# csm-kr/faster_rcnn_pytorch

Measured on AMD Instinct MI355X. Metric: train images/sec (VGG16 Faster R-CNN, 600x1000, bs=1/GPU), higher is better.
Workload: dtype f32; 1 GPU; VGG16 Faster R-CNN train step, synthetic 600x1000 frames, bs=1/GPU, HIP proposal/RoI path (N=20646 anchors, pre/post NMS 12000/2000, 128 RoIs, RoIPool 7x7 on 512x37x62); global_batch=1, parallelism=dp1, submission=eager (one launch per kernel), sampling=device-philox

## Files before the change

faster_rcnn_pytorch_amd/_lib.py:

```python
import ctypes as C
import os

_HERE = os.path.dirname(os.path.abspath(__file__))
LIB_PATH = os.environ.get("FRCNN_HIP_LIB") or os.path.join(_HERE, "lib", "libfrcnn_hip.so")

OK = 0
ABI_VERSION = 7
HT_ERR_PERM_LENGTH, HT_ERR_PERM_RANGE, HT_ERR_UPSTREAM_ABORT, HT_ERR_SHORT = 1, 2, 4, 8
HT_ERR_GT_COUNT = RPN_ERR_GT_COUNT = 16
OP_TOPK, OP_NMS, OP_REGION_PROPOSAL, OP_RPN_TARGETS, OP_HEAD_TARGETS, OP_PREPROCESS, OP_HEAD_BWD, OP_RPN_CONV, OP_RPN_CONV_WGRAD, OP_RPN_CONV_F32 = 1, 2, 3, 4, 5, 6, 7, 8, 9, 10
OP_DETECT = 11
OP_EVAL = 12
OP_COCO_EVAL = 13
OP_EVAL_MERGE = 14
OP_COCO_EVAL_POOLED = 15
OP_DETECT_MERGE = 16
MERGE_COUNT_CLIPPED, MERGE_UPSTREAM_ABORT, MERGE_LABEL_RANGE, MERGE_CLASS_OVERFLOW, MERGE_OUTPUT_OVERFLOW = 1, 2, 4, 8, 16
MERGE_MAX_SETS, MERGE_MAX_CANDIDATES = 8, 2048
SOFT_NMS_HARD, SOFT_NMS_LINEAR, SOFT_NMS_GAUSSIAN = 0, 1, 2
EVAL_TP, EVAL_FP, EVAL_IGNORED = 1, 2, 3
EVAL_ERR_UPSTREAM_ABORT, EVAL_ERR_GT_OVERFLOW, EVAL_ERR_COUNT_RANGE, EVAL_ERR_LABEL_RANGE = 1, 2, 4, 8
EVAL_ERR_LEDGER_OVERFLOW = 16
EVAL_ERR_SHARD_TRUNCATED = 32
EVAL_MERGE_MAX_SHARDS = 64
SGD_CHUNK = 8192

_vp, _i, _i64, _f, _u64, _sz = C.c_void_p, C.c_int, C.c_int64, C.c_float, C.c_uint64, C.c_size_t

SIGNATURES = {
    "frcnn_abi_version": (_i, []),
    "frcnn_layout_check": (_i, []),
    "frcnn_layout_stamp": (_u64, []),
    "frcnn_last_error": (C.c_char_p, []),
    "frcnn_workspace_bytes": (_sz, [_i, _i64, _i64]),
    "frcnn_anchor_base_host": (_i, [_i, _vp, _i, _vp, _i, _vp]),
    "frcnn_tv_base_anchors_host": (_i, [_f, _vp, _i, _vp]),
    "frcnn_anchor_grid": (_i, [_i, _vp, _vp, _vp, _vp, _vp, _i, _f, _f, _vp, _i64, _vp]),
    "frcnn_box_codec": (_i, [_i, _vp, _vp, _i64, _vp, _vp]),
    "frcnn_pairwise_iou": (_i, [_vp, _i64, _vp, _i64, _f, _vp, _vp]),
    "frcnn_proposal_prologue": (_i, [_vp, _vp, _vp, _i64, _f, _vp, _vp, _vp]),
    "frcnn_topk_sorted": (_i, [_vp, _vp, _i64, _i64, _vp, _vp, _vp, _vp, _vp, _sz, _vp]),
    "frcnn_argsort_desc": (_i, [_vp, _vp, _i64, _vp, _vp, _vp, _vp, _vp, _sz, _vp]),
    "frcnn_nms": (_i, [_vp, _vp, _i64, _f, _i64, _vp, _vp, _vp, _vp, _sz, _vp]),
    "frcnn_nms_classed": (_i, [_vp, _vp, _vp, _i64, _f, _i64, _vp, _vp, _vp, _vp, _sz, _vp]),
    "frcnn_region_proposal": (_i, [_vp, _vp, _vp, _i64, _i, _i, _i, _vp, _i, _f, _f, _f, _i64, _f, _i64, _vp, _i, _vp, _vp, _vp, _vp, _sz, _vp]),
    "frcnn_rpn_head_tail_fwd": (_i, [_vp, _i, _i64, _vp, _vp, _vp, _i, _vp, _vp, _i, _vp, _vp, _vp]),
    "frcnn_rpn_head_tail_ml_fwd": (_i, [_vp, _i, _i, _i, _vp, _i, _vp, _vp, _vp, _i, _vp, _vp, _i, _vp, _vp, _vp]),
    "frcnn_rpn_head_tail_ml_bwd": (_i, [_vp, _vp, _i, _i, _vp, _i, _vp, _vp, _i, _vp, _i, _vp, _vp, _vp, _vp, _vp, _vp, _vp, _vp, _sz, _vp]),
    "frcnn_rpn_conv_head_fwd": (_i, [_vp, _vp, _vp, _vp, _i, _i, _vp, _vp, _vp, _vp, _i, _vp, _vp, _i, _vp, _vp, _vp, _sz, _vp]),
    "frcnn_rpn_conv_bwd_data": (_i, [_vp, _vp, _vp, _vp, _i, _i, _vp, _vp, _sz, _vp]),
    "frcnn_rpn_conv_wgrad": (_i, [_vp, _vp, _vp, _vp, _i, _i, _vp, _vp, _sz, _vp]),
    "frcnn_rpn_conv3x3_f32_workspace": (_sz, [_vp, _vp, _i, _i]),
    "frcnn_gemm_nt_f32_workspace": (_sz, []),
    "frcnn_gemm_nt_f32": (_i, [_vp, _vp, _vp, _i, _i, _i, _i, _vp, _sz, _vp]),
    "frcnn_affine_act_fwd": (_i, [_vp, _vp, _vp, _vp, _vp, _i, _i, _i, _vp]),
    "frcnn_affine_act_bwd": (_i, [_vp, _vp, _vp, _vp, _vp, _i, _i, _i, _vp]),
    "frcnn_affine_act_fwd_mixed": (_i, [_vp, _i, _vp, _vp, _i, _vp, _vp, _vp, _i, _i, _i, _vp]),
    "frcnn_affine_act_bwd_mixed": (_i, [_vp, _i, _vp, _vp, _vp, _vp, _i, _vp, _i, _i, _i, _vp]),
    "frcnn_conv3x3_c3_fwd": (_i, [_vp, _vp, _i, _i, _i, _vp, _vp, _i, _vp, _vp]),
    "frcnn_conv3x3_c3_wgrad_workspace": (_sz, [_i, _i]),
    "frcnn_conv3x3_c3_wgrad": (_i, [_vp, _vp, _i, _i, _i, _vp, _vp, _vp, _vp, _sz, _vp]),
    "frcnn_conv3x3_f32_workspace": (_sz, [_vp, _vp, _i, _i, _i]),
    "frcnn_conv3x3_f32_xt_floats": (_sz, [_vp, _vp, _i, _i]),
    "frcnn_conv3x3_f32_relu_bits_words": (_sz, [_vp, _vp, _i, _i]),
    "frcnn_conv3x3_f32_u_floats": (_sz, [_vp, _vp, _i, _i, _i]),
    "frcnn_conv3x3_f32_products": (_i, [_i]),
    "frcnn_conv3x3_f32_fwd": (_i, [_vp, _vp, _vp, _vp, _i, _i, _i, _vp, _vp, _i, _vp, _vp, _vp, _vp, _sz, _vp]),
    "frcnn_conv3x3_f32_tile_size": (_i, [_vp, _vp, _i]),
    "frcnn_conv3x3_f32_supported": (_i, [_vp, _vp, _i, _i, _i, _i]),
    "frcnn_conv3x3_f32_plan": (_i, [_vp, _vp, _i, _i, _i, _vp, _i]),
    "frcnn_conv3x3_f32_bwd_data": (_i, [_vp, _vp, _vp, _vp, _vp, _i, _i, _i, _vp, _vp, _i, _vp, _i, _vp, _sz, _vp]),
    "frcnn_conv3x3_f32_wgrad": (_i, [_vp, _vp, _vp, _vp, _vp, _i, _i, _i, _vp, _vp, _vp, _i, _vp, _vp, _sz, _vp]),
    "frcnn_conv3x3_f32_bwd": (_i, [_vp, _vp, _vp, _vp, _vp, _i, _i, _i, _vp, _vp, _i, _vp, _vp, _vp, _vp, _vp, _sz, _vp]),
    "frcnn_rpn_conv3x3_f32_fwd": (_i, [_vp, _vp, _vp, _vp, _i, _i, _vp, _vp, _sz, _vp]),
    "frcnn_rpn_conv3x3_f32_bwd_data": (_i, [_vp, _vp, _vp, _vp, _i, _i, _vp, _vp, _sz, _vp]),
    "frcnn_rpn_conv3x3_f32_wgrad": (_i, [_vp, _vp, _vp, _vp, _i, _i, _vp, _vp, _sz, _vp]),
    "frcnn_rpn_targets": (_i, [_i, _vp, _i64, _vp, _i64, _vp, _i64, _vp, _i64, _u64, _u64, _vp, _vp, _vp, _vp, _vp, _sz, _vp]),
    "frcnn_head_targets": (_i, [_i, _vp, _vp, _i64, _vp, _vp, _i64, _i64, _i64, _i64, _vp, _i64, _vp, _i64, _u64, _u64, _vp,
                                _vp, _vp, _vp, _vp, _vp, _vp, _vp]),
    "frcnn_rpn_targets_n": (_i, [_i, _vp, _i64, _vp, _i64, _vp, _vp, _i64, _vp, _i64, _u64, _u64, _vp, _vp, _vp, _vp, _vp, _sz, _vp]),
    "frcnn_head_targets_n": (_i, [_i, _vp, _vp, _i64, _vp, _vp, _i64, _vp, _i64, _i64, _i64, _vp, _i64, _vp, _i64, _u64, _u64, _vp,
                                  _vp, _vp, _vp, _vp, _vp, _vp, _vp, _vp]),
    "frcnn_roi_pool_fwd": (_i, [_vp, _i, _i, _i, _vp, _i64, _i, _i, _f, _vp, _vp, _vp]),
    "frcnn_roi_pool_bwd": (_i, [_vp, _vp, _i64, _i, _i, _i, _i, _i, _vp, _vp]),
    "frcnn_roi_pool_fwd_a16": (_i, [_vp, _i, _i, _i, _vp, _i64, _f, _vp, _vp, _vp]),
    "frcnn_roi_pool_bwd_a16": (_i, [_vp, _vp, _vp, _f, _i64, _i, _i, _i, _vp, _vp]),
    "frcnn_roi_pool_plan": (_i, [_i, _i, _i, _i64, _i, _i, _i, _i, _vp, _i]),
    "frcnn_roi_level_map": (_i, [_vp, _i64, _i, _i, _f, _i, _f, _vp, _vp]),
    "frcnn_ms_roi_align_fwd": (_i, [_vp, _vp, _vp, _vp, _i, _i, _vp, _i64, _i, _i, _i, _i, _i, _f, _i, _vp, _vp, _vp, _vp]),
    "frcnn_roi_scale_order": (_i, [_vp, _i64, _vp, _vp, _vp, _vp, _i, _i, _i, _f, _i, _vp, _vp, _vp, _vp]),
    "frcnn_ms_roi_align_bwd": (_i, [_vp, _vp, _vp, _vp, _vp, _i, _i, _vp, _i64, _i, _i, _i, _i, _i, _f, _i, _vp, _sz, _vp]),
    "frcnn_ms_roi_align_bwd_workspace": (_sz, [_vp, _vp, _i, _i, _i64]),
    "frcnn_detection_loss": (_i, [_vp, _vp, _vp, _vp, _i64, _vp, _vp, _vp, _vp, _i64, _i, _vp, _vp, _vp, _vp, _vp, _vp, _sz, _vp]),
    "frcnn_detect_postprocess": (_i, [_vp, _vp, _vp, _vp, _i64, _i, _f, _vp, _f, _vp, _vp, _vp, _vp, _vp, _vp, _vp, _sz, _vp]),
    "frcnn_detect_merge": (_i, [_i, _vp, _vp, _vp, _vp, _vp, _vp, _i, _f, _f, _f, _vp, _vp, _vp, _vp, _vp, _vp, _i64, _vp, _sz, _vp]),
    "frcnn_detect_merge_soft": (_i, [_i, _vp, _vp, _vp, _vp, _vp, _vp, _i, _f, _f, _f, _i, _f, _f, _vp, _vp, _vp, _vp, _vp, _vp, _i64, _vp, _sz, _vp]),
    "frcnn_eval_update": (_i, [_vp, _vp, _vp, _vp, _i64, _vp, _vp, _vp, _vp, _i64, _vp, _vp, _i, _i, _vp, _vp, _vp, _vp, _vp, _vp, _i64, _vp, _vp,
                                _vp, _sz, _vp]),
    "frcnn_eval_average_precision": (_i, [_vp, _vp, _vp, _i64, _vp, _i, _i, _vp, _vp, _vp, _vp, _sz, _vp]),
    "frcnn_coco_eval_update": (_i, [_vp, _vp, _vp, _vp, _i64, _vp, _vp, _vp, _vp, _vp, _i64, _vp, _vp, _i, _i, _i, _vp, _vp, _vp, _vp, _vp, _vp, _i64,
                                     _vp, _vp, _vp, _sz, _vp]),
    "frcnn_coco_eval_update_pooled": (_i, [_vp, _vp, _vp, _vp, _i64, _vp, _vp, _vp, _vp, _vp, _i64, _vp, _vp, _i, _i, _i, _vp, _vp, _vp, _vp, _vp, _vp,
                                            _i64, _vp, _vp, _vp, _sz, _vp]),
    "frcnn_coco_eval_accumulate": (_i, [_vp, _vp, _vp, _vp, _i64, _vp, _vp, _i, _i, _i, _i, _i, _i, _vp, _vp, _vp, _sz, _vp]),
    "frcnn_eval_ledger_append": (_i, [_vp, _vp, _vp, _i64, _vp, _vp, _vp, _vp, _vp, _i64, _vp, _vp, _vp]),
    "frcnn_eval_merge": (_i, [_i, _i64, _i64, _i, _i64] + [_vp] * 11 + [_vp] * 5 + [_i64] + [_vp] * 3 + [_i64] + [_vp] * 6 + [_vp, _sz, _vp]),
    "frcnn_preprocess_image": (_i, [_vp, _i, _i, _i, _i, _i, _i, _i, _vp, _vp, _vp, _vp, _vp, _sz, _vp]),
    "frcnn_preprocess_boxes": (_i, [_vp, _i64, _i, _i, _i, _i, _i, _vp, _vp]),
    "frcnn_mosaic_workspace": (_sz, [_vp, _i, _i]),
    "frcnn_mosaic": (_i, [_vp, _vp, _i, _i, _vp, _vp, _vp, _vp, _vp, _vp, _vp, _vp, _vp, _vp, _sz, _vp]),
    "frcnn_photometric_workspace": (_sz, [_i, _i]),
# ... 106 lines not shown
```

faster_rcnn_pytorch_amd/csrc/conv_c3.hip:

```cpp
#include "frcnn_common.h"
#include "frcnn_dev.h"
#include "frcnn_internal.h"
#include "frcnn_layout.h"
FRCNN_LAYOUT_STAMP(conv_c3);

#define C3_TW 256

__global__ __launch_bounds__(256) void conv3x3_c3_fwd_kernel(const float *__restrict__ x, float *__restrict__ y, int H, int W, int Cout,
                                                             const float *__restrict__ w, const float *__restrict__ bias, int relu,
                                                             unsigned long long *__restrict__ bits)
{
    __shared__ float s[9][C3_TW + 4];
    extern __shared__ __attribute__((aligned(16))) float sw[];
    const int row = blockIdx.y, x0 = blockIdx.x * C3_TW, tid = threadIdx.x;
    for (int e = tid; e < Cout * 28; e += 256) {
        const int co = e / 28, k = e - co * 28;
        sw[e] = k < 27 ? w[(size_t)co * 27 + k] : (bias ? bias[co] : 0.0f);
    }
    {
        float v[10];
#pragma unroll
        for (int j = 0; j < 10; ++j) {
            const int e = tid + 256 * j, r = e / (C3_TW + 2), q = e - r * (C3_TW + 2), ci = r / 3, ky = r - 3 * ci, yy = row - 1 + ky, xx = x0 - 1 + q;
            v[j] = (r < 9 && yy >= 0 && yy < H && xx >= 0 && xx < W) ? x[((size_t)ci * H + yy) * W + xx] : 0.0f;
        }
#pragma unroll
        for (int j = 0; j < 10; ++j) {
            const int e = tid + 256 * j, r = e / (C3_TW + 2), q = e - r * (C3_TW + 2);
            if (r < 9) s[r][q] = v[j];
        }
    }
    __syncthreads();
    const int xx = x0 + tid;
    if (xx >= W) return;
    float v[27];
#pragma unroll
    for (int r = 0; r < 9; ++r)
#pragma unroll
        for (int kx = 0; kx < 3; ++kx) v[r * 3 + kx] = s[r][tid + kx];
    float *yo = y + (size_t)row * W + xx;
    const size_t plane = (size_t)H * W;
    unsigned long long word = 0;
    for (int c2 = 0; c2 < Cout; c2 += 2) {
        const bool two = c2 + 1 < Cout;
        const float4 *w0 = (const float4 *)&sw[c2 * 28], *w1 = (const float4 *)&sw[(two ? c2 + 1 : c2) * 28];
        float acc0 = sw[c2 * 28 + 27], acc1 = sw[(two ? c2 + 1 : c2) * 28 + 27];
#pragma unroll
        for (int q = 0; q < 7; ++q) {
            const float4 a = w0[q], c = w1[q];
            const float aw[4] = {a.x, a.y, a.z, a.w}, cw[4] = {c.x, c.y, c.z, c.w};
#pragma unroll
            for (int e = 0; e < 4; ++e)
                if (q * 4 + e < 27) { acc0 = fmaf(aw[e], v[q * 4 + e], acc0); acc1 = fmaf(cw[e], v[q * 4 + e], acc1); }
        }
#pragma unroll
        for (int j = 0; j < 2; ++j) {
            const int co = c2 + j;
            if (co < Cout) {
                const float pre = j ? acc1 : acc0, o = relu && pre < 0.0f ? 0.0f : pre;
                yo[(size_t)co * plane] = o;
                word |= o > 0.0f ? 1ull << (co & 63) : 0ull;
                if (bits && ((co & 63) == 63 || co == Cout - 1)) { bits[(size_t)(co >> 6) * plane + (size_t)row * W + xx] = word; word = 0; }
            }
        }
    }
}

#define C3_WAVES 8
#define C3_CPW 4
template <bool BITS>
__global__ __launch_bounds__(64 * C3_WAVES) void conv3x3_c3_wgrad_kernel(const float *__restrict__ x, const float *__restrict__ dy, int H, int W, int Cout,
                                                                       const unsigned long long *__restrict__ bits, float *__restrict__ part, int rows)
{
    extern __shared__ float s[];
    const int tid = threadIdx.x, lane = tid & 63, wave = tid >> 6, ws = W + 2, NT = 64 * C3_WAVES;
    const int co0 = (blockIdx.y * C3_WAVES + wave) * C3_CPW;
    const size_t plane = (size_t)H * W;
    typedef float c3_f32x2 __attribute__((ext_vector_type(2)));
    c3_f32x2 acc[C3_CPW][14];
#pragma unroll
    for (int j = 0; j < C3_CPW; ++j)
#pragma unroll
        for (int k = 0; k < 14; ++k) acc[j][k] = (c3_f32x2){0.0f, 0.0f};
    const int r0 = blockIdx.x * rows, nrow = min(rows, H - r0), RS = rows + 2, n_el = 3 * RS * ws;
    for (int base = tid; base < n_el; base += NT * 8) {
        float v[8];
#pragma unroll
        for (int j = 0; j < 8; ++j) {
            const int e = base + NT * j, rr = e / ws, q = e - rr * ws, ci = rr / RS, ry = rr - RS * ci, yy = r0 - 1 + ry, xx = q - 1;
            v[j] = (e < n_el && yy >= 0 && yy < H && xx >= 0 && xx < W) ? x[((size_t)ci * H + yy) * W + xx] : 0.0f;
        }
#pragma unroll
        for (int j = 0; j < 8; ++j) {
            const int e = base + NT * j;
            if (e < n_el) s[e] = v[j];
        }
    }
    __syncthreads();
    if (co0 >= Cout) return;
    const int nxb = (W + 255) / 256;
    auto load = [&](int ry, int xb, float (&gq)[4][C3_CPW], unsigned (&mq)[4]) {
        const float *g0 = dy + (size_t)co0 * plane + (size_t)(r0 + ry) * W;
        const unsigned *b0 = BITS ? (const unsigned *)(bits + (size_t)(co0 >> 6) * plane + (size_t)(r0 + ry) * W) + ((co0 & 63) >> 5) : nullptr;
#pragma unroll
        for (int i = 0; i < 4; ++i) {
            const int xc = min(xb + 64 * i + lane, W - 1);
            mq[i] = BITS ? b0[2 * xc] : ~0u;
#pragma unroll
            for (int j = 0; j < C3_CPW; ++j) gq[i][j] = g0[(size_t)j * plane + xc];
        }
    };
    float g[4][C3_CPW];
    unsigned mb[4];
    load(0, 0, g, mb);
    for (int ry = 0, xbi = 0;;) {
        const int xb = xbi * 256;
        int ry2 = ry, xbi2 = xbi + 1;
        if (xbi2 == nxb) { xbi2 = 0; ++ry2; }
        const bool more = ry2 < nrow;
        float gn[4][C3_CPW];
        unsigned mn[4];
        if (more) load(ry2, xbi2 * 256, gn, mn);
#pragma unroll
        for (int i = 0; i < 4; ++i) {
            const int xx = xb + 64 * i + lane;
            if (xb + 64 * i < W) {
                float v[27];
                const int xc = xx < W ? xx : W - 1;
#pragma unroll
                for (int r = 0; r < 9; ++r)
#pragma unroll
                    for (int kx = 0; kx < 3; ++kx) v[r * 3 + kx] = s[((r / 3) * RS + ry + r % 3) * ws + xc + kx];
#pragma unroll
                for (int j = 0; j < C3_CPW; ++j) {
                    const float gg = (xx < W && (!BITS || ((mb[i] >> ((co0 & 31) + j)) & 1u))) ? g[i][j] : 0.0f;
#pragma unroll
                    for (int k = 0; k < 14; ++k) {
                        const c3_f32x2 vv = {v[2 * k], k < 13 ? v[2 * k + 1] : 1.0f}, g2 = {gg, gg};
                        acc[j][k] = __builtin_elementwise_fma(g2, vv, acc[j][k]);
                    }
                }
            }
        }
        if (!more) break;
#pragma unroll
        for (int i = 0; i < 4; ++i) {
            mb[i] = mn[i];
#pragma unroll
            for (int j = 0; j < C3_CPW; ++j) g[i][j] = gn[i][j];
        }
        ry = ry2; xbi = xbi2;
    }
#pragma unroll
    for (int j = 0; j < C3_CPW; ++j)
#pragma unroll
        for (int k = 0; k < 28; ++k) {
            const float t = wave_sum_dpp(acc[j][k >> 1][k & 1]);
            if (lane == 63) part[((size_t)blockIdx.x * Cout + co0 + j) * 28 + k] = t;
        }
}

__global__ __launch_bounds__(256) void conv3x3_c3_wgrad_finalize_kernel(const float *__restrict__ part, int H, int Cout, float *__restrict__ dw,
                                                                        float *__restrict__ db)
{
    const int o = blockIdx.x * 256 + threadIdx.x;
    if (o >= Cout * 28) return;
    const size_t stride = (size_t)Cout * 28;
    float t = 0.0f;
    int r = 0;
    for (; r + 8 <= H; r += 8) {
        float v[8];
#pragma unroll
        for (int j = 0; j < 8; ++j) v[j] = part[(size_t)(r + j) * stride + o];
#pragma unroll
        for (int j = 0; j < 8; ++j) t += v[j];
    }
    for (; r < H; ++r) t += part[(size_t)r * stride + o];
    const int co = o / 28, k = o - co * 28;
    if (k < 27) dw[(size_t)co * 27 + k] = t;
    else if (db) db[co] = t;
}

static int c3_check(const void *x, const void *y, int H, int W, int Cout, const void *w, const char *what)
{
    FRCNN_REQUIRE(x && y && w, "%s: NULL pointer", what);
    FRCNN_REQUIRE(H > 0 && W > 0 && Cout > 0 && Cout <= 256 && (long long)H * W * Cout < (1ll << 31), "%s: bad size %d x %d x %d", what, Cout, H, W);
    return FRCNN_OK;
}

FRCNN_EXPORT int frcnn_conv3x3_c3_fwd(const float *x_dev, float *y_dev, int H, int W, int Cout, const float *w_dev, const float *bias_dev, int relu,
                                      unsigned long long *relu_bits_dev, void *stream)
{
    int rc = c3_check(x_dev, y_dev, H, W, Cout, w_dev, "conv3x3_c3_fwd");
    if (rc) return rc;
    FRCNN_LAUNCH(conv3x3_c3_fwd_kernel, dim3((unsigned)((W + C3_TW - 1) / C3_TW), (unsigned)H), dim3(256), (size_t)Cout * 28 * sizeof(float), (hipStream_t)stream, x_dev, y_dev, H, W, Cout,
                 w_dev, bias_dev, relu, relu_bits_dev);
    FRCNN_CHECK_LAUNCH("conv3x3_c3_fwd_kernel");
    return FRCNN_OK;
}

FRCNN_EXPORT size_t frcnn_conv3x3_c3_wgrad_workspace(int H, int Cout)
{
    return (H > 0 && Cout > 0) ? (size_t)H * Cout * 28 * sizeof(float) : 0;
}

FRCNN_EXPORT int frcnn_conv3x3_c3_wgrad(const float *x_dev, const float *dy_dev, int H, int W, int Cout, const unsigned long long *relu_bits_dev,
                                        float *dw_dev, float *dbias_dev, void *workspace, size_t workspace_bytes, void *stream)
{
    int rc = c3_check(x_dev, dy_dev, H, W, Cout, dw_dev, "conv3x3_c3_wgrad");
    if (rc) return rc;
    FRCNN_REQUIRE(dw_dev && workspace, "conv3x3_c3_wgrad: NULL pointer");
    if (Cout % 4 != 0 || W > 1700)
        return frcnn_set_error(FRCNN_ERR_UNSUPPORTED, "conv3x3_c3_wgrad: Cout = %d must be a multiple of 4 and W = %d at most 1700", Cout, W);
    if (workspace_bytes < frcnn_conv3x3_c3_wgrad_workspace(H, Cout))
        return frcnn_set_error(FRCNN_ERR_WORKSPACE, "conv3x3_c3_wgrad: workspace %zu < %zu bytes", workspace_bytes, frcnn_conv3x3_c3_wgrad_workspace(H, Cout));
    hipStream_t s = (hipStream_t)stream;
    float *part = (float *)workspace;
    const int groups = (Cout + C3_CPW * C3_WAVES - 1) / (C3_CPW * C3_WAVES);
    int cus = 256, dev = 0;
    if (hipGetDevice(&dev) == hipSuccess) (void)hipDeviceGetAttribute(&cus, hipDeviceAttributeMultiprocessorCount, dev);
    const int fit = (int)((150 * 1024) / (12 * (size_t)(W + 2))) - 2;
    const int rows = std::max(1, std::min(fit, (int)(((long long)H * groups + cus - 1) / cus)));
    const int nb = (H + rows - 1) / rows;
    const dim3 wg((unsigned)nb, (unsigned)groups);
    const size_t wl = (size_t)3 * (rows + 2) * (W + 2) * sizeof(float);
    if (relu_bits_dev) (void)hipFuncSetAttribute((const void *)conv3x3_c3_wgrad_kernel<true>, hipFuncAttributeMaxDynamicSharedMemorySize, (int)wl);
    else (void)hipFuncSetAttribute((const void *)conv3x3_c3_wgrad_kernel<false>, hipFuncAttributeMaxDynamicSharedMemorySize, (int)wl);
    if (relu_bits_dev) FRCNN_LAUNCH(conv3x3_c3_wgrad_kernel<true>, wg, dim3(64 * C3_WAVES), wl, s, x_dev, dy_dev, H, W, Cout, relu_bits_dev, part, rows);
    else FRCNN_LAUNCH(conv3x3_c3_wgrad_kernel<false>, wg, dim3(64 * C3_WAVES), wl, s, x_dev, dy_dev, H, W, Cout, relu_bits_dev, part, rows);
    FRCNN_CHECK_LAUNCH("conv3x3_c3_wgrad_kernel");
    FRCNN_LAUNCH(conv3x3_c3_wgrad_finalize_kernel, dim3((unsigned)((Cout * 28 + 255) / 256)), dim3(256), 0, s, part, nb, Cout, dw_dev, dbias_dev);
    FRCNN_CHECK_LAUNCH("conv3x3_c3_wgrad_finalize_kernel");
    return FRCNN_OK;
}
```

faster_rcnn_pytorch_amd/ops.py:

```python
import collections
import ctypes as C

import numpy as np
import torch

from . import _lib
from ._lib import check, lib


def _stream():
    return C.c_void_p(torch.cuda.current_stream().cuda_stream)


def _ptr(t):
    return C.c_void_p(0 if t is None else t.data_ptr())


def _req(t, dtype=torch.float32, name="tensor"):
    if not isinstance(t, torch.Tensor):
        raise TypeError("%s must be a torch.Tensor" % name)
    if not t.is_cuda:
        raise RuntimeError("%s is on %s: the frcnn ops run only on a HIP device (no CPU fallback)" % (name, t.device))
    if t.dtype != dtype:
        raise TypeError("%s must be %s, got %s" % (name, dtype, t.dtype))
# ... 1238 lines not shown
        if x.dtype not in (torch.bfloat16, torch.float32) or not x.is_cuda:
            raise ValueError("affine_act_mixed: x must be a bf16 or fp32 HIP tensor")
        x = x.contiguous()
        Cc, HW = int(x.shape[1]), int(x.shape[2] * x.shape[3])
        if res is not None:
            res = _req(res, name="res")
            if res.shape != x.shape:
                raise ValueError("affine_act_mixed: residual and input differ in shape")
        ctx.set_materialize_grads(False)
        y = torch.empty_like(x, dtype=torch.bfloat16 if out_bf16 else torch.float32)
        twin = torch.empty_like(x, dtype=torch.bfloat16) if want_twin else None
        with torch.cuda.device(x.device):
            check(lib.frcnn_affine_act_fwd_mixed(_ptr(x), 1 if x.dtype == torch.bfloat16 else 0, _ptr(res), _ptr(y), 1 if out_bf16 else 0, _ptr(twin),
                                                 _ptr(scale), _ptr(shift), Cc, HW, 1 if relu else 0, _stream()), "affine_act_fwd_mixed")
        _affine_trace("affine_act_fwd_mixed_kernel", x, res, y, twin, scale, shift)
        ctx.relu, ctx.has_res, ctx.x_bf16, ctx.twin = bool(relu), res is not None, x.dtype == torch.bfloat16, bool(want_twin)
        ctx.save_for_backward(scale, y if relu else None)
        if want_twin:
            return y, twin
        return y

    @staticmethod
    def backward(ctx, g, g2=None):
        scale, y = ctx.saved_tensors
        need_x, need_r = ctx.needs_input_grad[5], ctx.has_res and ctx.needs_input_grad[6]
        if not need_x and not need_r:
            return None, None, None, None, None, None, None
        if g is None and g2 is None:
            return None, None, None, None, None, None, None
        if g is None:
            g = torch.zeros_like(g2, dtype=torch.float32)
        g = g.contiguous()
        if g2 is not None:
            g2 = g2.contiguous()
        Cc, HW = int(g.shape[1]), int(g.shape[2] * g.shape[3])
        dx = torch.empty_like(g, dtype=torch.bfloat16 if ctx.x_bf16 else torch.float32)
        dres = torch.empty_like(g, dtype=torch.float32) if (need_r and (ctx.relu or g2 is not None or g.dtype != torch.float32)) else None
        with torch.cuda.device(g.device):
            check(lib.frcnn_affine_act_bwd_mixed(_ptr(g), 1 if g.dtype == torch.bfloat16 else 0, _ptr(g2), _ptr(y), _ptr(scale), _ptr(dx),
                                                 1 if ctx.x_bf16 else 0, _ptr(dres), Cc, HW, 1 if ctx.relu else 0, _stream()), "affine_act_bwd_mixed")
        _affine_trace("affine_act_bwd_mixed_kernel", g, g2, y, dx, dres, scale)
        return None, None, None, None, None, (dx if need_x else None), ((dres if dres is not None else g) if need_r else None)


def affine_act_mixed(x, scale, shift, res=None, relu=False, out_bf16=False, twin=False):
    return _AffineActMixedFn.apply(bool(relu), bool(out_bf16), bool(twin), scale.reshape(-1), shift.reshape(-1), x, res)


def affine_act_mixed_supported(x):
    return (x.is_cuda and x.dtype in (torch.bfloat16, torch.float32) and x.dim() == 4 and x.shape[0] == 1 and torch.is_autocast_enabled()
            and torch.get_autocast_dtype("cuda") == torch.bfloat16)


def conv3x3_c3_fwd(x, w, bias=None, relu=False, want_bits=False):
    x, w = _req(x, name="x"), _req(w, name="w")
    if x.dim() != 4 or x.shape[0] != 1 or x.shape[1] != 3 or w.dim() != 4 or tuple(w.shape[1:]) != (3, 3, 3):
        raise ValueError("conv3x3_c3: x must be [1,3,h,w] and w [Cout,3,3,3]")
    Cout, H, W = int(w.shape[0]), int(x.shape[2]), int(x.shape[3])
    if bias is not None:
        bias = _req(bias, name="bias")
    y = torch.empty((1, Cout, H, W), dtype=torch.float32, device=x.device)
    bits = torch.empty(((Cout + 63) // 64, H, W), dtype=torch.int64, device=x.device) if want_bits else None
    with torch.cuda.device(x.device):
        check(lib.frcnn_conv3x3_c3_fwd(_ptr(x), _ptr(y), H, W, Cout, _ptr(w), _ptr(bias), 1 if relu else 0, _ptr(bits), _stream()), "conv3x3_c3_fwd")
    return (y, bits) if want_bits else y


def conv3x3_c3_wgrad(x, dy, relu_bits=None, want_bias=True):
    x, dy = _req(x, name="x"), _req(dy, name="dy")
    Cout, H, W = int(dy.shape[1]), int(x.shape[2]), int(x.shape[3])
    if x.dim() != 4 or x.shape[0] != 1 or x.shape[1] != 3 or tuple(dy.shape) != (1, Cout, H, W):
        raise ValueError("conv3x3_c3_wgrad: x must be [1,3,h,w] and dy [1,Cout,h,w]")
    if relu_bits is not None:
        relu_bits = _req(relu_bits, torch.int64, "relu_bits")
        if tuple(relu_bits.shape) != ((Cout + 63) // 64, H, W):
            raise ValueError("conv3x3_c3_wgrad: relu_bits does not belong to these shapes")
    dw = torch.empty((Cout, 3, 3, 3), dtype=torch.float32, device=x.device)
    db = torch.empty((Cout,), dtype=torch.float32, device=x.device) if want_bias else None
    ws = _workspace(x.device, int(lib.frcnn_conv3x3_c3_wgrad_workspace(H, Cout)))
    with torch.cuda.device(x.device):
        check(lib.frcnn_conv3x3_c3_wgrad(_ptr(x), _ptr(dy), H, W, Cout, _ptr(relu_bits), _ptr(dw), _ptr(db), _ptr(ws), ws.numel(), _stream()), "conv3x3_c3_wgrad")
    return dw, db


class _Conv3x3C3Fn(torch.autograd.Function):

    @staticmethod
    def forward(ctx, relu, w, bias, x):
        grads = ctx.needs_input_grad[1] or (bias is not None and ctx.needs_input_grad[2])
        if relu and grads:
            y, bits = conv3x3_c3_fwd(x, w, bias, True, want_bits=True)
        else:
            y, bits = conv3x3_c3_fwd(x, w, bias, relu), None
        ctx.has_bias = bias is not None
        ctx.save_for_backward(x, bits)
        return y

    @staticmethod
    def backward(ctx, g):
        x, bits = ctx.saved_tensors
        if ctx.needs_input_grad[3]:
            raise RuntimeError("conv3x3_c3: no input gradient (the input is the image)")
        dw, db = conv3x3_c3_wgrad(x, g.contiguous(), bits, want_bias=ctx.has_bias)
        return None, dw, db, None


# ... 453 lines not shown
```

include/frcnn_hip.h:

```cpp
#ifndef FRCNN_HIP_H
#define FRCNN_HIP_H

#include <stddef.h>
#include <stdint.h>

#ifdef __cplusplus
extern "C" {
#endif

#define FRCNN_ABI_VERSION 7

typedef enum {
    FRCNN_OK = 0,
    FRCNN_ERR_INVALID_ARG = -1,
    FRCNN_ERR_UNSUPPORTED = -2,
    FRCNN_ERR_WORKSPACE = -3,
    FRCNN_ERR_LAUNCH = -4
} frcnn_status;

typedef enum { FRCNN_DTYPE_F32 = 0, FRCNN_DTYPE_BF16 = 1 } frcnn_dtype;

typedef enum {
    FRCNN_OP_TOPK = 1,
    FRCNN_OP_NMS = 2,
// ... 76 lines not shown
                               float *db3, void *workspace, size_t workspace_bytes, void *stream);

int frcnn_rpn_conv_head_fwd(const void *const *feat_levels_bf16, void *const *raw_levels_bf16, const int *H_host, const int *W_host, int n_levels,
                            int C, const float *w3, const float *b3, const float *w_cls, const float *b_cls, int n_cls, const float *w_reg,
                            const float *b_reg, int n_reg, float *out_cls, float *out_reg, void *workspace, size_t workspace_bytes, void *stream);

int frcnn_rpn_conv_bwd_data(const void *const *d_raw_levels_bf16, void *const *d_feat_levels_bf16, const int *H_host, const int *W_host, int n_levels,
                            int C, const float *w3, void *workspace, size_t workspace_bytes, void *stream);

int frcnn_rpn_conv_wgrad(const void *const *feat_levels_bf16, const void *const *d_raw_levels_bf16, const int *H_host, const int *W_host, int n_levels,
                         int C, float *dw3, void *workspace, size_t workspace_bytes, void *stream);

size_t frcnn_rpn_conv3x3_f32_workspace(const int *H_host, const int *W_host, int n_levels, int C);
int frcnn_rpn_conv3x3_f32_fwd(const float *const *feat_levels, float *const *out_levels, const int *H_host, const int *W_host, int n_levels, int C,
                              const float *w3, void *workspace, size_t workspace_bytes, void *stream);
int frcnn_rpn_conv3x3_f32_bwd_data(const float *const *d_out_levels, float *const *d_feat_levels, const int *H_host, const int *W_host, int n_levels,
                                   int C, const float *w3, void *workspace, size_t workspace_bytes, void *stream);
int frcnn_rpn_conv3x3_f32_wgrad(const float *const *feat_levels, const float *const *d_out_levels, const int *H_host, const int *W_host, int n_levels,
                                int C, float *dw3, void *workspace, size_t workspace_bytes, void *stream);

size_t frcnn_conv3x3_f32_workspace(const int *H_host, const int *W_host, int n_levels, int Cin, int Cout);
size_t frcnn_conv3x3_f32_xt_floats(const int *H_host, const int *W_host, int n_levels, int Cin);
size_t frcnn_conv3x3_f32_u_floats(const int *H_host, const int *W_host, int n_levels, int Cin, int Cout);
size_t frcnn_conv3x3_f32_relu_bits_words(const int *H_host, const int *W_host, int n_levels, int Cout);
int frcnn_conv3x3_f32_tile_size(const int *H_host, const int *W_host, int n_levels);
int frcnn_conv3x3_f32_supported(const int *H_host, const int *W_host, int n_levels, int Cin, int Cout, int need_grads);
#define FRCNN_CONV_SCHED_STREAM_K 0
#define FRCNN_CONV_SCHED_WHOLE_RANGES 1
#define FRCNN_CONV_SCHED_ONE_TILE 2
#define FRCNN_CONV_SCHED_FUSED_OUT64 3
#define FRCNN_CONV_PLAN_MAX_LEVELS 8
#define FRCNN_CONV_PLAN_HEAD 8
#define FRCNN_CONV_PLAN_PRODUCT 10
#define FRCNN_CONV_PLAN_STRIPS (2 + 4 * FRCNN_CONV_PLAN_MAX_LEVELS)
#define FRCNN_CONV_PLAN_INTS (FRCNN_CONV_PLAN_HEAD + 3 * FRCNN_CONV_PLAN_PRODUCT + 2 * FRCNN_CONV_PLAN_STRIPS)
int frcnn_conv3x3_f32_plan(const int *H_host, const int *W_host, int n_levels, int Cin, int Cout, int *plan_host, int plan_len);
int frcnn_conv3x3_f32_products(int mode);
int frcnn_conv3x3_f32_fwd(const float *const *x_levels, float *const *y_levels, const int *H_host, const int *W_host, int n_levels, int Cin, int Cout,
                          const float *w, const float *bias, int relu, unsigned short *relu_bits, float *x_transformed, float *u_rotated, void *workspace,
                          size_t workspace_bytes, void *stream);
int frcnn_conv3x3_f32_bwd_data(const float *const *dy_levels, const unsigned short *relu_bits, float *const *dx_levels, const int *H_host, const int *W_host,
                               int n_levels, int Cin, int Cout, const float *w, const float *u_rotated, int pooled, float *dy_transformed,
                               int want_bias_partials, void *workspace, size_t workspace_bytes, void *stream);
int frcnn_conv3x3_f32_wgrad(const float *const *x_levels, const float *const *dy_levels, const unsigned short *relu_bits, const int *H_host, const int *W_host,
                            int n_levels, int Cin, int Cout, float *dw, float *dbias, const float *x_transformed, int pooled, const float *dy_transformed,
                            void *workspace, size_t workspace_bytes, void *stream);
int frcnn_conv3x3_f32_bwd(const float *const *dy_levels, const unsigned short *relu_bits, float *const *dx_levels, const int *H_host, const int *W_host,
                          int n_levels, int Cin, int Cout, const float *w, const float *u_rotated, int pooled, const float *x_transformed,
                          float *dy_transformed, float *dw, float *dbias, void *workspace, size_t workspace_bytes, void *stream);

size_t frcnn_gemm_nt_f32_workspace(void);
int frcnn_gemm_nt_f32(const float *A, const float *B, float *O, int M, int N, int K, int splits, void *workspace, size_t workspace_bytes, void *stream);

int frcnn_conv3x3_c3_fwd(const float *x, float *y, int H, int W, int Cout, const float *w, const float *bias, int relu, unsigned long long *relu_bits,
                         void *stream);
size_t frcnn_conv3x3_c3_wgrad_workspace(int H, int Cout);
int frcnn_conv3x3_c3_wgrad(const float *x, const float *dy, int H, int W, int Cout, const unsigned long long *relu_bits, float *dw, float *dbias,
                           void *workspace, size_t workspace_bytes, void *stream);

int frcnn_affine_act_fwd(const float *x, const float *res, float *y, const float *scale, const float *shift, int C, int HW, int relu, void *stream);
int frcnn_affine_act_bwd(const float *g, const float *y, const float *scale, float *dx, float *dres, int C, int HW, int relu, void *stream);
int frcnn_affine_act_fwd_mixed(const void *x, int x_dtype, const float *res, void *y, int y_dtype, void *twin_bf16, const float *scale, const float *shift,
                               int C, int HW, int relu, void *stream);
int frcnn_affine_act_bwd_mixed(const void *g, int g_dtype, const void *g2_bf16, const void *y, const float *scale, void *dx, int dx_dtype, float *dres,
                               int C, int HW, int relu, void *stream);

int frcnn_rpn_targets(int variant, const float *anchors , int64_t N, const float *gt , int64_t G,
                      const int64_t *perm_pos, int64_t n_perm_pos, const int64_t *perm_neg, int64_t n_perm_neg,
                      uint64_t seed, uint64_t offset, uint64_t *philox_state_dev ,
                      int64_t *out_cls , float *out_reg , int32_t *out_counts ,
                      void *workspace, size_t workspace_bytes, void *stream);
#define FRCNN_RPN_ERR_GT_COUNT 16
int frcnn_rpn_targets_n(int variant, const float *anchors , int64_t N, const float *gt , int64_t G_cap,
                        const int32_t *n_gt_dev ,
                        const int64_t *perm_pos, int64_t n_perm_pos, const int64_t *perm_neg, int64_t n_perm_neg,
                        uint64_t seed, uint64_t offset, uint64_t *philox_state_dev ,
                        int64_t *out_cls , float *out_reg , int32_t *out_counts ,
                        void *workspace, size_t workspace_bytes, void *stream);

#define FRCNN_HT_ERR_PERM_LENGTH 1
#define FRCNN_HT_ERR_PERM_RANGE 2
#define FRCNN_HT_ERR_UPSTREAM_ABORT 4
#define FRCNN_HT_ERR_SHORT 8
int frcnn_head_targets(int variant, const float *rois, const int32_t *n_rois_dev, int64_t P_cap,
                       const float *gt, const int64_t *gt_label, int64_t G,
                       int64_t label_offset, int64_t max_pos, int64_t total,
                       const int64_t *perm_pos, int64_t n_perm_pos, const int64_t *perm_neg, int64_t n_perm_neg,
                       uint64_t seed, uint64_t offset, uint64_t *philox_state_dev ,
                       int64_t *out_cls , float *out_reg , float *out_rois ,
                       int64_t *out_keep_index , int32_t *out_counts ,
                       int32_t *sticky_status , void *stream);
#define FRCNN_HT_ERR_GT_COUNT 16
int frcnn_head_targets_n(int variant, const float *rois, const int32_t *n_rois_dev, int64_t P_cap,
                         const float *gt , const int64_t *gt_label , int64_t G_cap,
                         const int32_t *n_gt_dev ,
                         int64_t label_offset, int64_t max_pos, int64_t total,
                         const int64_t *perm_pos, int64_t n_perm_pos, const int64_t *perm_neg, int64_t n_perm_neg,
                         uint64_t seed, uint64_t offset, uint64_t *philox_state_dev,
                         int64_t *out_cls , float *out_reg , float *out_rois ,
                         int64_t *out_keep_index , int32_t *out_counts ,
                         int32_t *sticky_status , int32_t *empty_dev , void *stream);

int frcnn_roi_pool_fwd(const float *feat, int C, int H, int W, const float *rois, int64_t R, int PH, int PW,
                       float spatial_scale, float *out , int32_t *argmax , void *stream);
int frcnn_roi_pool_bwd(const float *grad_out, const int32_t *argmax, int64_t R, int C, int H, int W, int PH, int PW,
                       float *grad_feat, void *stream);
// ... 267 lines not shown
```

Before: 149.0 images/s.

## Add multi-pixel first-conv forward and deeper-prefetch wgrad variants behind a runtime switch

The 3-input-channel first conv forward now lets each thread compute two adjacent pixels. This reuses loaded weights and input windows across pixels and issues vectorized input, output and ReLU-bit stores. The wgrad kernel gets a variant that prefetches two pieces of dy ahead, using triple-buffered registers, and stages its shared input in larger batches. Both are chosen by default through a runtime variant flag that an env var or API can override. The change also adds compile-time ablation macros, which are off by default, and it raises register pressure.

```diff
diff --git a/faster_rcnn_pytorch_amd/_lib.py b/faster_rcnn_pytorch_amd/_lib.py
--- a/faster_rcnn_pytorch_amd/_lib.py
+++ b/faster_rcnn_pytorch_amd/_lib.py
@@ -57,6 +57,7 @@
     "frcnn_affine_act_bwd": (_i, [_vp, _vp, _vp, _vp, _vp, _i, _i, _i, _vp]),
     "frcnn_affine_act_fwd_mixed": (_i, [_vp, _i, _vp, _vp, _i, _vp, _vp, _vp, _i, _i, _i, _vp]),
     "frcnn_affine_act_bwd_mixed": (_i, [_vp, _i, _vp, _vp, _vp, _vp, _i, _vp, _i, _i, _i, _vp]),
+    "frcnn_conv3x3_c3_variant": (_i, [_i]),
     "frcnn_conv3x3_c3_fwd": (_i, [_vp, _vp, _i, _i, _i, _vp, _vp, _i, _vp, _vp]),
     "frcnn_conv3x3_c3_wgrad_workspace": (_sz, [_i, _i]),
     "frcnn_conv3x3_c3_wgrad": (_i, [_vp, _vp, _i, _i, _i, _vp, _vp, _vp, _vp, _sz, _vp]),
diff --git a/faster_rcnn_pytorch_amd/csrc/conv_c3.hip b/faster_rcnn_pytorch_amd/csrc/conv_c3.hip
--- a/faster_rcnn_pytorch_amd/csrc/conv_c3.hip
+++ b/faster_rcnn_pytorch_amd/csrc/conv_c3.hip
@@ -2,13 +2,22 @@
 #include "frcnn_dev.h"
 #include "frcnn_internal.h"
 #include "frcnn_layout.h"
+#include <algorithm>
+#include <atomic>
+#include <cstdlib>
+#include <cstring>
 FRCNN_LAYOUT_STAMP(conv_c3);
 
 #define C3_TW 256
 
-__global__ __launch_bounds__(256) void conv3x3_c3_fwd_kernel(const float *__restrict__ x, float *__restrict__ y, int H, int W, int Cout,
-                                                             const float *__restrict__ w, const float *__restrict__ bias, int relu,
-                                                             unsigned long long *__restrict__ bits)
+#ifndef C3_ABL
+#define C3_ABL 0
+#endif
+#define C3_ABL_STORE(o) (!(C3_ABL & 2) || (o) == 1.2345e30f)
+
+__device__ __forceinline__ void c3_fwd_px1(const float *__restrict__ x, float *__restrict__ y, int H, int W, int Cout,
+                                           const float *__restrict__ w, const float *__restrict__ bias, int relu,
+                                           unsigned long long *__restrict__ bits)
 {
     __shared__ float s[9][C3_TW + 4];
     extern __shared__ __attribute__((aligned(16))) float sw[];
@@ -47,7 +56,15 @@
         float acc0 = sw[c2 * 28 + 27], acc1 = sw[(two ? c2 + 1 : c2) * 28 + 27];
 #pragma unroll
         for (int q = 0; q < 7; ++q) {
+#if C3_ABL & 4
+            if (q >= 0) continue;
+#endif
+#if C3_ABL & 1
+            const float fa = (float)(relu + c2 + q);
+            const float4 a = make_float4(fa, fa + 1.0f, fa + 2.0f, fa + 3.0f), c = make_float4(fa + 4.0f, fa + 5.0f, fa + 6.0f, fa + 7.0f);
+#else
             const float4 a = w0[q], c = w1[q];
+#endif
             const float aw[4] = {a.x, a.y, a.z, a.w}, cw[4] = {c.x, c.y, c.z, c.w};
 #pragma unroll
             for (int e = 0; e < 4; ++e)
@@ -58,7 +75,7 @@
             const int co = c2 + j;
             if (co < Cout) {
                 const float pre = j ? acc1 : acc0, o = relu && pre < 0.0f ? 0.0f : pre;
-                yo[(size_t)co * plane] = o;
+                if (C3_ABL_STORE(o)) yo[(size_t)co * plane] = o;
                 word |= o > 0.0f ? 1ull << (co & 63) : 0ull;
                 if (bits && ((co & 63) == 63 || co == Cout - 1)) { bits[(size_t)(co >> 6) * plane + (size_t)row * W + xx] = word; word = 0; }
             }
@@ -66,11 +83,127 @@
     }
 }
 
+#define C3_PX 2
+template <int PX> struct c3_vec;
+template <> struct c3_vec<2> { typedef float2 f; };
+template <> struct c3_vec<4> { typedef float4 f; };
+template <int PX>
+__device__ __forceinline__ void c3_fwd_pxn(const float *__restrict__ x, float *__restrict__ y, int H, int W, int Cout,
+                                           const float *__restrict__ w, const float *__restrict__ bias, int relu,
+                                           unsigned long long *__restrict__ bits)
+{
+    typedef typename c3_vec<PX>::f vec;
+    constexpr int TW = 256 * PX, WS = TW + 8;
+    __shared__ __attribute__((aligned(16))) float sp[9][WS];
+    extern __shared__ __attribute__((aligned(16))) float sw[];
+    const int row = blockIdx.y, x0 = blockIdx.x * TW, tid = threadIdx.x;
+    for (int e = tid; e < Cout * 28; e += 256) {
+        const int co = e / 28, k = e - co * 28;
+        sw[e] = k < 27 ? w[(size_t)co * 27 + k] : (bias ? bias[co] : 0.0f);
+    }
+    const int xx = x0 + PX * tid;
+    {
+        vec v[9];
+#pragma unroll
+        for (int r = 0; r < 9; ++r) {
+            const int ci = r / 3, yy = row - 1 + r % 3;
+            v[r] = vec{};
+            if (yy >= 0 && yy < H && xx < W) v[r] = *(const vec *)&x[((size_t)ci * H + yy) * W + xx];
+        }
+        float hv = 0.0f;
+        const int hr = tid >> 1, hx = (tid & 1) ? x0 + TW : x0 - 1;
+        if (tid < 18) {
+            const int ci = hr / 3, yy = row - 1 + hr % 3;
+            if (yy >= 0 && yy < H && hx >= 0 && hx < W) hv = x[((size_t)ci * H + yy) * W + hx];
+        }
+#pragma unroll
+        for (int r = 0; r < 9; ++r) *(vec *)&sp[r][4 + PX * tid] = v[r];
+        if (tid < 18) sp[hr][(tid & 1) ? 4 + TW : 3] = hv;
+    }
+    __syncthreads();
+    if (xx >= W) return;
+    float v[9][PX + 2];
+#pragma unroll
+    for (int r = 0; r < 9; ++r) {
+        const vec m = *(const vec *)&sp[r][4 + PX * tid];
+        v[r][0] = sp[r][3 + PX * tid];
+        v[r][PX + 1] = sp[r][4 + PX + PX * tid];
+        v[r][1] = m.x; v[r][2] = m.y;
+        if constexpr (PX == 4) { v[r][3] = m.z; v[r][4] = m.w; }
+    }
+    const size_t plane = (size_t)H * W, pix = (size_t)row * W + xx;
+    float *yo = y + pix;
+    unsigned long long word[PX];
+#pragma unroll
+    for (int p = 0; p < PX; ++p) word[p] = 0;
+    for (int c2 = 0; c2 < Cout; c2 += 2) {
+        const bool two = c2 + 1 < Cout;
+        const float4 *w0 = (const float4 *)&sw[c2 * 28], *w1 = (const float4 *)&sw[(two ? c2 + 1 : c2) * 28];
+        float acc0[PX], acc1[PX];
+#pragma unroll
+        for (int p = 0; p < PX; ++p) { acc0[p] = sw[c2 * 28 + 27]; acc1[p] = sw[(two ? c2 + 1 : c2) * 28 + 27]; }
+#pragma unroll
+        for (int q = 0; q < 7; ++q) {
+#if C3_ABL & 4
+            if (q >= 0) continue;
+#endif
+#if C3_ABL & 1
+            const float fa = (float)(relu + c2 + q);
+            const float4 a = make_float4(fa, fa + 1.0f, fa + 2.0f, fa + 3.0f), c = make_float4(fa + 4.0f, fa + 5.0f, fa + 6.0f, fa + 7.0f);
+#else
+            const float4 a = w0[q], c = w1[q];
+#endif
+            const float aw[4] = {a.x, a.y, a.z, a.w}, cw[4] = {c.x, c.y, c.z, c.w};
+#pragma unroll
+            for (int e = 0; e < 4; ++e)
+                if (q * 4 + e < 27) {
+                    const int k = q * 4 + e, r = k / 3, kx = k - 3 * r;
+#pragma unroll
+                    for (int p = 0; p < PX; ++p) { acc0[p] = fmaf(aw[e], v[r][p + kx], acc0[p]); acc1[p] = fmaf(cw[e], v[r][p + kx], acc1[p]); }
+                }
+        }
+#pragma unroll
+        for (int j = 0; j < 2; ++j) {
+            const int co = c2 + j;
+            if (co < Cout) {
+                float o[PX];
+#pragma unroll
+                for (int p = 0; p < PX; ++p) {
+                    const float pre = j ? acc1[p] : acc0[p];
+                    o[p] = relu && pre < 0.0f ? 0.0f : pre;
+                    word[p] |= o[p] > 0.0f ? 1ull << (co & 63) : 0ull;
+                }
+                if (C3_ABL_STORE(o[0])) {
+                    if constexpr (PX == 4) *(float4 *)&yo[(size_t)co * plane] = make_float4(o[0], o[1], o[2], o[3]);
+                    else *(float2 *)&yo[(size_t)co * plane] = make_float2(o[0], o[1]);
+                }
+                if (bits && ((co & 63) == 63 || co == Cout - 1)) {
+                    ulonglong2 *bo = (ulonglong2 *)&bits[(size_t)(co >> 6) * plane + pix];
+#pragma unroll
+                    for (int p = 0; p < PX; p += 2) bo[p >> 1] = make_ulonglong2(word[p], word[p + 1]);
+#pragma unroll
+                    for (int p = 0; p < PX; ++p) word[p] = 0;
+                }
+            }
+        }
+    }
+}
+
+template <int PX>
+__global__ __launch_bounds__(256) void conv3x3_c3_fwd_kernel(const float *__restrict__ x, float *__restrict__ y, int H, int W, int Cout,
+                                                             const float *__restrict__ w, const float *__restrict__ bias, int relu,
+                                                             unsigned long long *__restrict__ bits)
+{
+    if constexpr (PX == 1) c3_fwd_px1(x, y, H, W, Cout, w, bias, relu, bits);
+    else c3_fwd_pxn<PX>(x, y, H, W, Cout, w, bias, relu, bits);
+}
+
 #define C3_WAVES 8
 #define C3_CPW 4
+#define C3_STAGE 24
 template <bool BITS>
-__global__ __launch_bounds__(64 * C3_WAVES) void conv3x3_c3_wgrad_kernel(const float *__restrict__ x, const float *__restrict__ dy, int H, int W, int Cout,
-                                                                       const unsigned long long *__restrict__ bits, float *__restrict__ part, int rows)
+__device__ __forceinline__ void c3_wgrad_ahead1(const float *__restrict__ x, const float *__restrict__ dy, int H, int W, int Cout,
+                                                const unsigned long long *__restrict__ bits, float *__restrict__ part, int rows)
 {
     extern __shared__ float s[];
     const int tid = threadIdx.x, lane = tid & 63, wave = tid >> 6, ws = W + 2, NT = 64 * C3_WAVES;
@@ -120,7 +253,11 @@
         const bool more = ry2 < nrow;
         float gn[4][C3_CPW];
         unsigned mn[4];
+#if C3_ABL & 8
+        for (int i = 0; i < 4; ++i) { mn[i] = mb[i]; for (int j = 0; j < C3_CPW; ++j) gn[i][j] = g[i][j]; }
+#else
         if (more) load(ry2, xbi2 * 256, gn, mn);
+#endif
 #pragma unroll
         for (int i = 0; i < 4; ++i) {
             const int xx = xb + 64 * i + lane;
@@ -158,6 +295,118 @@
             const float t = wave_sum_dpp(acc[j][k >> 1][k & 1]);
             if (lane == 63) part[((size_t)blockIdx.x * Cout + co0 + j) * 28 + k] = t;
         }
+}
+
+template <bool BITS>
+__device__ __forceinline__ void c3_wgrad_ahead2(const float *__restrict__ x, const float *__restrict__ dy, int H, int W, int Cout,
+                                                const unsigned long long *__restrict__ bits, float *__restrict__ part, int rows)
+{
+    extern __shared__ float s[];
+    const int tid = threadIdx.x, lane = tid & 63, wave = tid >> 6, ws = W + 2, NT = 64 * C3_WAVES;
+    const int co0 = (blockIdx.y * C3_WAVES + wave) * C3_CPW;
+    const size_t plane = (size_t)H * W;
+    typedef float c3_f32x2 __attribute__((ext_vector_type(2)));
+    c3_f32x2 acc[C3_CPW][14];
+#pragma unroll
+    for (int j = 0; j < C3_CPW; ++j)
+#pragma unroll
+        for (int k = 0; k < 14; ++k) acc[j][k] = (c3_f32x2){0.0f, 0.0f};
+    const int r0 = blockIdx.x * rows, nrow = min(rows, H - r0), RS = rows + 2, n_el = 3 * RS * ws;
+    {
+        int rr = tid / ws, q = tid - rr * ws;
+        const int drr = NT / ws, dq = NT - drr * ws;
+        for (int base = tid; base < n_el; base += NT * C3_STAGE) {
+            float v[C3_STAGE];
+#pragma unroll
+            for (int j = 0; j < C3_STAGE; ++j) {
+                const int e = base + NT * j, ci = rr >= 2 * RS ? 2 : rr >= RS ? 1 : 0, yy = r0 - 1 + rr - RS * ci, xx = q - 1;
+                v[j] = (e < n_el && yy >= 0 && yy < H && xx >= 0 && xx < W) ? x[((size_t)ci * H + yy) * W + xx] : 0.0f;
+                rr += drr; q += dq;
+                if (q >= ws) { q -= ws; ++rr; }
+            }
+#pragma unroll
+            for (int j = 0; j < C3_STAGE; ++j) {
+                const int e = base + NT * j;
+                if (e < n_el) s[e] = v[j];
+            }
+        }
+    }
+    __syncthreads();
+    if (co0 >= Cout) return;
+    const int nxb = (W + 255) / 256, n = nrow * nxb;
+    auto load = [&](int ry, int xb, float (&gq)[4][C3_CPW], unsigned (&mq)[4]) {
+        const float *g0 = dy + (size_t)co0 * plane + (size_t)(r0 + ry) * W;
+        const unsigned *b0 = BITS ? (const unsigned *)(bits + (size_t)(co0 >> 6) * plane + (size_t)(r0 + ry) * W) + ((co0 & 63) >> 5) : nullptr;
+#pragma unroll
+        for (int i = 0; i < 4; ++i) {
+            const int xc = min(xb + 64 * i + lane, W - 1);
+            mq[i] = BITS ? b0[2 * xc] : ~0u;
+#pragma unroll
+            for (int j = 0; j < C3_CPW; ++j) gq[i][j] = g0[(size_t)j * plane + xc];
+        }
+    };
+    int lry = 0, lxb = 0;
+    auto load_next = [&](float (&gq)[4][C3_CPW], unsigned (&mq)[4]) {
+        load(lry, lxb * 256, gq, mq);
+        if (lxb + 1 < nxb) ++lxb;
+        else if (lry + 1 < nrow) { lxb = 0; ++lry; }
+    };
+    int ry = 0, xbi = 0;
+    auto sum_piece = [&](const float (&g)[4][C3_CPW], const unsigned (&mb)[4]) {
+        const int xb = xbi * 256;
+#pragma unroll
+        for (int i = 0; i < 4; ++i) {
+            const int xx = xb + 64 * i + lane;
+            if (xb + 64 * i < W) {
+                float v[27];
+                const int xc = xx < W ? xx : W - 1;
+#pragma unroll
+                for (int r = 0; r < 9; ++r)
+#pragma unroll
+                    for (int kx = 0; kx < 3; ++kx) v[r * 3 + kx] = s[((r / 3) * RS + ry + r % 3) * ws + xc + kx];
+#pragma unroll
+                for (int j = 0; j < C3_CPW; ++j) {
+                    const float gg = (xx < W && (!BITS || ((mb[i] >> ((co0 & 31) + j)) & 1u))) ? g[i][j] : 0.0f;
+#pragma unroll
+                    for (int k = 0; k < 14; ++k) {
+                        const c3_f32x2 vv = {v[2 * k], k < 13 ? v[2 * k + 1] : 1.0f}, gp = {gg, gg};
+                        acc[j][k] = __builtin_elementwise_fma(gp, vv, acc[j][k]);
+                    }
+                }
+            }
+        }
+        if (++xbi == nxb) { xbi = 0; ++ry; }
+    };
+    float ga[4][C3_CPW], gb[4][C3_CPW], gc[4][C3_CPW];
+    unsigned ma[4], mb[4], mc[4];
+    load_next(ga, ma);
+    load_next(gb, mb);
+    for (int p = 0;;) {
+        load_next(gc, mc);
+        sum_piece(ga, ma);
+        if (++p == n) break;
+        load_next(ga, ma);
+        sum_piece(gb, mb);
+        if (++p == n) break;
+        load_next(gb, mb);
+        sum_piece(gc, mc);
+        if (++p == n) break;
+    }
+#pragma unroll
+    for (int j = 0; j < C3_CPW; ++j)
+#pragma unroll
+        for (int k = 0; k < 28; ++k) {
+            const float t = wave_sum_dpp(acc[j][k >> 1][k & 1]);
+            if (lane == 63) part[((size_t)blockIdx.x * Cout + co0 + j) * 28 + k] = t;
+        }
+}
+
+template <bool BITS, int AHEAD>
+__global__ __launch_bounds__(64 * C3_WAVES) void conv3x3_c3_wgrad_kernel(const float *__restrict__ x, const float *__restrict__ dy, int H, int W, int Cout,
+                                                                       const unsigned long long *__restrict__ bits, float *__restrict__ part, int rows)
+{
+    if constexpr (AHEAD == 1) c3_wgrad_ahead1<BITS>(x, dy, H, W, Cout, bits, part, rows);
+    else c3_wgrad_ahead2<BITS>(x, dy, H, W, Cout, bits, part, rows);
 }
 
 __global__ __launch_bounds__(256) void conv3x3_c3_wgrad_finalize_kernel(const float *__restrict__ part, int H, int Cout, float *__restrict__ dw,
@@ -181,6 +430,13 @@
     else if (db) db[co] = t;
 }
 
+static std::atomic<int> g_c3_variant{[] { const char *e = getenv("FRCNN_CONV_C3_VARIANT"); return (e && !strcmp(e, "0")) ? 0 : 1; }()};
+FRCNN_EXPORT int frcnn_conv3x3_c3_variant(int variant)
+{
+    if (variant < 0) return g_c3_variant.load();
+    return g_c3_variant.exchange(variant ? 1 : 0);
+}
+
 static int c3_check(const void *x, const void *y, int H, int W, int Cout, const void *w, const char *what)
 {
     FRCNN_REQUIRE(x && y && w, "%s: NULL pointer", what);
@@ -193,8 +449,13 @@
 {
     int rc = c3_check(x_dev, y_dev, H, W, Cout, w_dev, "conv3x3_c3_fwd");
     if (rc) return rc;
-    FRCNN_LAUNCH(conv3x3_c3_fwd_kernel, dim3((unsigned)((W + C3_TW - 1) / C3_TW), (unsigned)H), dim3(256), (size_t)Cout * 28 * sizeof(float), (hipStream_t)stream, x_dev, y_dev, H, W, Cout,
-                 w_dev, bias_dev, relu, relu_bits_dev);
+    const bool wide = g_c3_variant.load() != 0 && W % C3_PX == 0 && (((uintptr_t)x_dev | (uintptr_t)y_dev) & (4 * C3_PX - 1)) == 0 &&
+                      ((uintptr_t)relu_bits_dev & (8 * C3_PX - 1)) == 0;
+    const int tw = wide ? C3_TW * C3_PX : C3_TW;
+    const dim3 grid((unsigned)((W + tw - 1) / tw), (unsigned)H);
+    const size_t wl = (size_t)Cout * 28 * sizeof(float);
+    if (wide) FRCNN_LAUNCH(conv3x3_c3_fwd_kernel<C3_PX>, grid, dim3(256), wl, (hipStream_t)stream, x_dev, y_dev, H, W, Cout, w_dev, bias_dev, relu, relu_bits_dev);
+    else FRCNN_LAUNCH(conv3x3_c3_fwd_kernel<1>, grid, dim3(256), wl, (hipStream_t)stream, x_dev, y_dev, H, W, Cout, w_dev, bias_dev, relu, relu_bits_dev);
     FRCNN_CHECK_LAUNCH("conv3x3_c3_fwd_kernel");
     return FRCNN_OK;
 }
@@ -224,10 +485,14 @@
     const int nb = (H + rows - 1) / rows;
     const dim3 wg((unsigned)nb, (unsigned)groups);
     const size_t wl = (size_t)3 * (rows + 2) * (W + 2) * sizeof(float);
-    if (relu_bits_dev) (void)hipFuncSetAttribute((const void *)conv3x3_c3_wgrad_kernel<true>, hipFuncAttributeMaxDynamicSharedMemorySize, (int)wl);
-    else (void)hipFuncSetAttribute((const void *)conv3x3_c3_wgrad_kernel<false>, hipFuncAttributeMaxDynamicSharedMemorySize, (int)wl);
-    if (relu_bits_dev) FRCNN_LAUNCH(conv3x3_c3_wgrad_kernel<true>, wg, dim3(64 * C3_WAVES), wl, s, x_dev, dy_dev, H, W, Cout, relu_bits_dev, part, rows);
-    else FRCNN_LAUNCH(conv3x3_c3_wgrad_kernel<false>, wg, dim3(64 * C3_WAVES), wl, s, x_dev, dy_dev, H, W, Cout, relu_bits_dev, part, rows);
+    const bool ahead2 = g_c3_variant.load() != 0;
+#define C3_WGRAD_CASE(BITSv, AHEADv)                                                                                                                              \
+    if ((relu_bits_dev != nullptr) == BITSv && ahead2 == (AHEADv == 2)) {                                                                                         \
+        (void)hipFuncSetAttribute((const void *)conv3x3_c3_wgrad_kernel<BITSv, AHEADv>, hipFuncAttributeMaxDynamicSharedMemorySize, (int)wl);                     \
+        FRCNN_LAUNCH((conv3x3_c3_wgrad_kernel<BITSv, AHEADv>), wg, dim3(64 * C3_WAVES), wl, s, x_dev, dy_dev, H, W, Cout, relu_bits_dev, part, rows);             \
+    }
+    C3_WGRAD_CASE(true, 1) C3_WGRAD_CASE(false, 1) C3_WGRAD_CASE(true, 2) C3_WGRAD_CASE(false, 2)
+#undef C3_WGRAD_CASE
     FRCNN_CHECK_LAUNCH("conv3x3_c3_wgrad_kernel");
     FRCNN_LAUNCH(conv3x3_c3_wgrad_finalize_kernel, dim3((unsigned)((Cout * 28 + 255) / 256)), dim3(256), 0, s, part, nb, Cout, dw_dev, dbias_dev);
     FRCNN_CHECK_LAUNCH("conv3x3_c3_wgrad_finalize_kernel");
diff --git a/faster_rcnn_pytorch_amd/ops.py b/faster_rcnn_pytorch_amd/ops.py
--- a/faster_rcnn_pytorch_amd/ops.py
+++ b/faster_rcnn_pytorch_amd/ops.py
@@ -1314,6 +1314,14 @@
             and torch.get_autocast_dtype("cuda") == torch.bfloat16)
 
 
+def conv3x3_c3_variant(variant=None):
+    if variant is None:
+        return int(lib.frcnn_conv3x3_c3_variant(-1))
+    if variant not in (0, 1):
+        raise ValueError("conv3x3_c3_variant: variant must be 0 or 1")
+    return int(lib.frcnn_conv3x3_c3_variant(int(variant)))
+
+
 def conv3x3_c3_fwd(x, w, bias=None, relu=False, want_bits=False):
     x, w = _req(x, name="x"), _req(w, name="w")
     if x.dim() != 4 or x.shape[0] != 1 or x.shape[1] != 3 or w.dim() != 4 or tuple(w.shape[1:]) != (3, 3, 3):
diff --git a/include/frcnn_hip.h b/include/frcnn_hip.h
--- a/include/frcnn_hip.h
+++ b/include/frcnn_hip.h
@@ -152,6 +152,7 @@
 size_t frcnn_gemm_nt_f32_workspace(void);
 int frcnn_gemm_nt_f32(const float *A, const float *B, float *O, int M, int N, int K, int splits, void *workspace, size_t workspace_bytes, void *stream);
 
+int frcnn_conv3x3_c3_variant(int variant);
 int frcnn_conv3x3_c3_fwd(const float *x, float *y, int H, int W, int Cout, const float *w, const float *bias, int relu, unsigned long long *relu_bits,
                          void *stream);
 size_t frcnn_conv3x3_c3_wgrad_workspace(int H, int Cout);
```

Result: no change. 148.8 images/s (-0.1%).
